# Sun-Sir/BSARec

Measured on AMD Instinct MI355X. Metric: train sequences/sec, ML-1M L=50 d=64 2-layer, higher is better.
Workload: dtype f32

## Files before the change

### bsarec_amd/csrc/fused_layer.h

```cpp
#pragma once
#include "common.h"
#include "kernels.h"
#include <type_traits>

#define FS 68
#define FU 260
#define FUSED_MAX_CB 8

struct FusedFwdP {
    const float* X; float* Xout;
    const float *sqrt_beta, *f_g, *f_b, *wq, *bq, *wk, *bk, *wv, *bv, *wo, *bo, *a_g, *a_b, *w1, *b1, *w2, *b2, *ff_g, *ff_b;
    const float* tw; const int* ids32;
    float *xhat_f, *rstd_f, *q, *k, *v, *probs, *ctx, *xhat_a, *rstd_a, *hmix, *u, *xhat_ff, *rstd_ff, *dsp;
    float* gp;
    int L, Lp, cb, heads;
    float alpha, oma, eps;
    DropP drop_f, drop_p, drop_o, drop_ff;
    float* trash;
    long long* stamps;
    const float *e_E, *e_pos, *e_g, *e_b; const int64_t* e_ids; GatherP e_gp; DropP e_drop; int e_V;
    float *e_X0, *e_xhat, *e_rstd; int* e_ids32;
    int xout_f32;
    const float* filter_cw;
};
// ... 568 lines not shown
        }
    }
    WFrag<MM, 32> wO;
    if constexpr (!FM) load_w<MM, 32>(R2_wo, wrow + 32 * grp, wO);
    lds_barrier();
    if constexpr (!FM) {
    {
        const int lr = tid >> 4, lc = (tid & 15) << 2;
#pragma unroll
        for (int r0 = 0; r0 < 64; r0 += 32) {
            const int r = r0 + lr;
            if (r < L) {
                const long e = (tok0 + r) * 64 + lc;
                ast4<BF>(R2_q, e, ld4(sQ + r * FS + lc));
                ast4<BF>(R2_k, e, ld4(sK + r * FS + lc));
                ast4<BF>(R2_v, e, f32x4{sVt[lc * FS + r], sVt[(lc + 1) * FS + r], sVt[(lc + 2) * FS + r], sVt[(lc + 3) * FS + r]});
            }
        }
    }

    STAMP(3);
    const auto R3_ctx = KARG(FusedFwdP, ctx);
    const auto R3_drop_p = KARG(FusedFwdP, drop_p);
    const auto R3_probs = KARG(FusedFwdP, probs);
    {
        const int nt = (L + 31) >> 5;
        const float sqrt_dh = sqrtf((float)DH);
        constexpr int NCT = (DH + 31) / 32;
        const int ncombo = heads * nt;
        const int pair = wave >> 1, kt = wave & 1;
        for (int c0 = 0; c0 < ncombo; c0 += 4) {
            const int combo = c0 + pair;
            const bool act = combo < ncombo && kt < nt;
            const int head = act ? combo / nt : 0, qt = act ? combo % nt : 0;
            const int query = 32 * qt + l31;
            f32x16 st;
#pragma unroll
            for (int r = 0; r < 16; ++r) st[r] = 0.f;
            float mx = -INFINITY;
            if (act) {
                mma_ll<MM, DH>(sK + (32 * kt + l31) * FS + head * DH + KH, sQ + query * FS + head * DH + KH, st);
#pragma unroll
                for (int r = 0; r < 16; ++r) {
                    const int key = 32 * kt + rho(r) + 4 * half;
                    float s = -INFINITY;
                    if (key < L) s = st[r] / sqrt_dh + ((key <= query && sIds[key] > 0) ? 0.0f : -10000.0f);
                    st[r] = s;
                    mx = fmaxf(mx, s);
                }
                mx = xor32_max(mx);
                sRed[(pair * 2 + kt) * 64 + lane] = mx;
            }
            lds_barrier();
            float sum = 0.f;
            if (act) {
                if (nt == 2) mx = fmaxf(mx, sRed[(pair * 2 + (kt ^ 1)) * 64 + lane]);
#pragma unroll
                for (int r = 0; r < 16; ++r) {
                    const int key = 32 * kt + rho(r) + 4 * half;
                    const float e = key < L ? __expf(st[r] - mx) : 0.f;
                    st[r] = e;
                    sum += e;
                }
                sum = xor32_sum(sum);
            }
            lds_barrier();
            if (act) sRed[(pair * 2 + kt) * 64 + lane] = sum;
            lds_barrier();
            if (act) {
                if (nt == 2) sum += sRed[(pair * 2 + (kt ^ 1)) * 64 + lane];
                const float inv = 1.0f / sum;
#pragma unroll
                for (int g = 0; g < 4; ++g) {
                    const int key0 = 32 * kt + 8 * g + 4 * half;
                    f32x4 p = {st[4 * g] * inv, st[4 * g + 1] * inv, st[4 * g + 2] * inv, st[4 * g + 3] * inv};
                    f32x4 m = {1.f, 1.f, 1.f, 1.f};
                    if (query < L && key0 < Lp) {
                        const long e = (((long)b * heads + head) * L + query) * Lp + key0;
                        ast4<BF>(R3_probs, e, p);
                        m = drop_mult4(R3_drop_p, dseed, (uint64_t)e >> 2);
                    }
                    p = p * m;
                    st[4 * g] = p.x; st[4 * g + 1] = p.y; st[4 * g + 2] = p.z; st[4 * g + 3] = p.w;
                }
                float* dstT = kt == 0 ? sC : sE;
#pragma unroll
                for (int ct = 0; ct < NCT; ++ct) {
                    f32x16 cacc;
#pragma unroll
                    for (int r = 0; r < 16; ++r) cacc[r] = 0.f;
                    const bool crow_ok = 32 * ct + l31 < DH;
                    const float* va = sVt + (head * DH + 32 * ct + (crow_ok ? l31 : 0)) * FS + 32 * kt + 4 * half;
                    if constexpr (MM != 0) {
#pragma unroll
                        for (int s2 = 0; s2 < 2; ++s2) {
                            f32x4 a0 = ld4(va + 16 * s2), a1 = ld4(va + 16 * s2 + 8);
                            if (!crow_ok) { a0 = f32x4{0, 0, 0, 0}; a1 = a0; }
                            if constexpr (MM == 1) {
                                const u32x4 pb = {pk_bf16(st[8 * s2], st[8 * s2 + 1]), pk_bf16(st[8 * s2 + 2], st[8 * s2 + 3]),
                                                  pk_bf16(st[8 * s2 + 4], st[8 * s2 + 5]), pk_bf16(st[8 * s2 + 6], st[8 * s2 + 7])};
                                cacc = mfma_bf16(pk8(a0, a1), pb, cacc);
                            } else {
                                cacc = mfma_x3(split3(a0, a1), split3(f32x4{st[8 * s2], st[8 * s2 + 1], st[8 * s2 + 2], st[8 * s2 + 3]},
                                                                      f32x4{st[8 * s2 + 4], st[8 * s2 + 5], st[8 * s2 + 6], st[8 * s2 + 7]}), cacc);
                            }
                        }
                    } else {
#pragma unroll
                    for (int g = 0; g < 4; ++g) {
                        f32x4 a = ld4(va + 8 * g);
                        if (!crow_ok) a = f32x4{0, 0, 0, 0};
#pragma unroll
                        for (int j = 0; j < 4; ++j)
                            cacc = __builtin_amdgcn_mfma_f32_32x32x2f32(a[j], st[4 * g + j], cacc, 0, 0, 0);
                    }
                    }
#pragma unroll
                    for (int g = 0; g < 4; ++g) {
                        const int c = 32 * ct + 8 * g + 4 * half;
                        if (c < DH)
                            st4(dstT + query * FS + head * DH + c, f32x4{cacc[4 * g], cacc[4 * g + 1], cacc[4 * g + 2], cacc[4 * g + 3]});
                    }
                }
            }
            lds_barrier();
        }
        {
            const int lr = tid >> 4, lc = (tid & 15) << 2;
#pragma unroll
            for (int r0 = 0; r0 < 64; r0 += 32) {
                const int r = r0 + lr;
                f32x4 v = {0, 0, 0, 0};
                if (r < 32 * nt) { v = ld4(sC + r * FS + lc); if (nt == 2) v += ld4(sE + r * FS + lc); }
                st4(sC + r * FS + lc, v);
                if (r < L) ast4<BF>(R3_ctx, (tok0 + r) * 64 + lc, v);
            }
        }
    }
    lds_barrier();
    }

    STAMP(4);
    const auto R4_a_b = KARG(FusedFwdP, a_b);
    const auto R4_a_g = KARG(FusedFwdP, a_g);
    const auto R4_alpha = KARG(FusedFwdP, alpha);
    const auto R4_bo = KARG(FusedFwdP, bo);
    const auto R4_drop_o = KARG(FusedFwdP, drop_o);
    const auto R4_eps = KARG(FusedFwdP, eps);
    const auto R4_hmix = KARG(FusedFwdP, hmix);
    const auto R4_oma = KARG(FusedFwdP, oma);
    const auto R4_rstd_a = KARG(FusedFwdP, rstd_a);
    const auto R4_w1 = KARG(FusedFwdP, w1);
    const auto R4_xhat_a = KARG(FusedFwdP, xhat_a);
    float ffn_bias[2];
    LnPre lnA;
    if constexpr (!FM) lnA = ln_pre(R4_bo, R4_a_g, R4_a_b, R4_drop_o, dseed, tok0);
    {
        load_w<MM, 64>(R4_w1, (long)(128 * grp + col) * 64 + KH, wA);
        ffn_bias[0] = gld(KARG(FusedFwdP, b1) + 128 * grp + col); ffn_bias[1] = gld(KARG(FusedFwdP, b1) + 128 * grp + 64 + col);
        if constexpr (!FM) {
        f32x16 acc;
#pragma unroll
        for (int r = 0; r < 16; ++r) acc[r] = 0.f;
        mma_w<MM, 32>(sC + arow + 32 * grp, wO, acc);
        float* part = grp == 0 ? sQ : sK;
#pragma unroll
        for (int r = 0; r < 16; ++r) part[(wm * 32 + rho(r) + 4 * half) * FS + col] = acc[r];
        }
    }
    if constexpr (!FM) {
    lds_barrier();
    ln_rows_64<true, BF>(lnA, sQ, sK, sX, R4_eps, sD, R4_alpha, R4_oma, tok0, L, sH, R4_hmix, R4_xhat_a, R4_rstd_a);
    lds_barrier();
    }

    STAMP(5);
    const auto R5_b1 = KARG(FusedFwdP, b1);
    const auto R5_u = KARG(FusedFwdP, u);
    const auto R5_w1 = KARG(FusedFwdP, w1);
    const auto R5_w2 = KARG(FusedFwdP, w2);
    {
        const float* sa = sH + arow;
#pragma unroll
        for (int i = 0; i < 2; ++i) {
            const int c256 = (2 * grp + i) * 64 + col;
            WFrag<MM, 64>& wcur = i ? wB : wA;
            WFrag<MM, 64>& wnxt = i ? wA : wB;
            if (i == 0) load_w<MM, 64>(R5_w1, (long)(c256 + 64) * 64 + KH, wnxt);
            else load_w<MM, 64>(R5_w2, (long)col * 256 + 128 * grp + KH, wnxt);
            f32x16 acc;
#pragma unroll
            for (int r = 0; r < 16; ++r) acc[r] = 0.f;
            mma_w<MM, 64>(sa, wcur, acc);
            const float bias = ffn_bias[i];
#pragma unroll
            for (int r = 0; r < 16; ++r) {
                const int row = wm * 32 + rho(r) + 4 * half;
                sU[row * FU + c256] = acc[r] + bias;
            }
        }
    }
    lds_barrier();

    STAMP(6);
    const auto R6_w2 = KARG(FusedFwdP, w2);
    const auto R6_u = KARG(FusedFwdP, u);
    const auto R6_gp = KARG(FusedFwdP, gp);
    const auto R7_b2 = KARG(FusedFwdP, b2);
    const auto R7_drop_ff = KARG(FusedFwdP, drop_ff);
    const auto R7_ff_b = KARG(FusedFwdP, ff_b);
    const auto R7_ff_g = KARG(FusedFwdP, ff_g);
    LnPre lnF;
    {
        for (int idx = tid; idx < 64 * 64; idx += 512) {
            const int r = idx >> 6, c4 = (idx & 63) << 2;
            const f32x4 v = ld4(sU + r * FU + c4);
            float g0, g1, g2, g3, p0, p1, p2, p3;
            gelu_both(v.x, g0, p0); gelu_both(v.y, g1, p1); gelu_both(v.z, g2, p2); gelu_both(v.w, g3, p3);
            const f32x4 g = {g0, g1, g2, g3}, gp = {p0, p1, p2, p3};
            if (r < L) { ast4<BF>(R6_u, (tok0 + r) * 256 + c4, g); ast4<BF>(R6_gp, (tok0 + r) * 256 + c4, gp); }
            st4(sU + r * FU + c4, g);
        }
        lds_barrier();
        lnF = ln_pre(R7_b2, R7_ff_g, R7_ff_b, R7_drop_ff, dseed, tok0);
        f32x16 acc;
#pragma unroll
        for (int r = 0; r < 16; ++r) acc[r] = 0.f;
        const float* sa = sU + (wm * 32 + l31) * FU + 128 * grp + KH;
        load_w<MM, 64>(R6_w2, (long)col * 256 + 128 * grp + 64 + KH, wB);
        mma_w<MM, 64>(sa, wA, acc);
        mma_w<MM, 64>(sa + 64, wB, acc);
        float* part = grp == 0 ? sX : sE;
#pragma unroll
        for (int r = 0; r < 16; ++r) part[(wm * 32 + rho(r) + 4 * half) * FS + col] = acc[r];
    }
    lds_barrier();
    STAMP(7);
    TopFwdRegs<BF> TR;
    TopFwdHelpRegs<BF> TH;
    if constexpr (TAIL) { if (wave < 4) top_fwd_prefetch<BF, KOFF, false>(TR); else top_fwd_help_prefetch<BF, KOFF>(TH); }
    const auto R7_Xout = KARG(FusedFwdP, Xout);
    const auto R7_eps = KARG(FusedFwdP, eps);
    const auto R7_rstd_ff = KARG(FusedFwdP, rstd_ff);
    const auto R7_xhat_ff = KARG(FusedFwdP, xhat_ff);
    ln_rows_64<false, BF>(lnF, sX, sE, sH, R7_eps, nullptr, 0.f, 1.f, tok0, L,
                          TAIL ? sD : nullptr, R7_Xout, R7_xhat_ff, R7_rstd_ff, KARG(FusedFwdP, xout_f32) != 0, TAIL);
    STAMP(8);
    if constexpr (TAIL) {
        lds_barrier();
        if (wave < 4) top_fwd_rest<DH, BF, KOFF, true>(TR, dseed, sD, sR, sR + TS, sR + 2 * TS, sTab, sSpec, sX, sIds);
        else top_fwd_help<DH, BF, KOFF>(TH, sD, sR, sR + TS, sX);
    }
}
#undef PTYPE

static inline size_t fused_fwd_smem_bytes() {
    return (size_t)(8 * 64 * FS + 2 * FUSED_MAX_CB * 128 + 512 + 64) * 4;
}

struct FusedBwdP {
    const float* dY; float* dX; const float* X;
    const float *sqrt_beta, *f_g, *wq, *wk, *wv, *wo, *a_g, *w1, *w2, *ff_g;
    const float* tw;
    const float *xhat_f, *rstd_f, *q, *k, *v, *probs, *xhat_a, *rstd_a, *u, *xhat_ff, *rstd_ff;
    const float* dh_slabs; int dh_nsplit; long dh_stride;
    float *dT, *dU, *dO, *dq, *dk, *dv;
    float *pg_ff, *pb_ff, *pg_a, *pb_a, *pg_f, *pb_f, *pbeta;
    int L, Lp, cb, heads;
    float alpha, oma;
    DropP drop_f, drop_p, drop_o, drop_ff;
    float* trash;
    long long* stamps;
    float* e_dz; const float *e_xhat, *e_rstd, *e_g; float *e_pg, *e_pb; DropP e_drop;
    const float* filter_cw; float* pcw;
    const float* e_dx_extra;
};


__device__ __forceinline__ void seq_partial_64(const f32x4& v, float* __restrict__ red, float* __restrict__ dst, float scale_by = 1.f,
                                               const float* __restrict__ mul = nullptr) {
    const int lr = threadIdx.x >> 4, lc = (threadIdx.x & 15) << 2;
    const int ng = blockDim.x >> 4;
    lds_barrier();
    st4(red + lr * 64 + lc, v);
    lds_barrier();
    if (threadIdx.x < 64) {
        float s = 0.f;
        for (int g = 0; g < ng; ++g) s += red[g * 64 + threadIdx.x];
        if (mul) s *= gld(mul + threadIdx.x);
        gst(dst + threadIdx.x, s * scale_by);
    }
}


template <int N>
__device__ __forceinline__ void seq_partials_64(const f32x4 (&v)[N], float* const (&red)[N], float* const (&dst)[N],
                                                float scale0 = 1.f, const float* __restrict__ mul0 = nullptr) {
    const int lr = threadIdx.x >> 4, lc = (threadIdx.x & 15) << 2;
    const int ng = blockDim.x >> 4;
    lds_barrier();
#pragma unroll
    for (int i = 0; i < N; ++i) st4(red[i] + lr * 64 + lc, v[i]);
    lds_barrier();
    const int i = threadIdx.x >> 6, c = threadIdx.x & 63;
    if (i < N) {
        const float* r = red[0];
        float* d = dst[0];
#pragma unroll
        for (int k = 1; k < N; ++k) if (i == k) { r = red[k]; d = dst[k]; }
        float s0 = 0.f, s1 = 0.f, s2 = 0.f, s3 = 0.f;
        for (int g = 0; g < ng; g += 4) {
            s0 += r[g * 64 + c]; s1 += r[(g + 1) * 64 + c]; s2 += r[(g + 2) * 64 + c]; s3 += r[(g + 3) * 64 + c];
        }
        float sum = (s0 + s1) + (s2 + s3);
        if (i == 0) { if (mul0) sum *= gld(mul0 + c); sum *= scale0; }
        gst(d + c, sum);
    }
}

template <int DH, bool BF, class HEADP, bool X3 = false, bool FM = false>
__global__ void __launch_bounds__(512) __attribute__((amdgpu_waves_per_eu(2, 2)))
fused_layer_bwd_kernel(const FusedBwdP P_unused, const HEADP H_unused) {
#define PTYPE FusedBwdP
    static_assert(!(BF && X3), "x3 products work on fp32 tensors");
    constexpr int MM = X3 ? 2 : (BF ? 1 : 0);
    static_assert(!FM || (!BF && !X3 && !IsTail<HEADP>::value), "the FMLPRec block runs in fp32, without a top-block head");
    constexpr bool HEAD = IsTail<HEADP>::value;
    constexpr unsigned KOFF = (unsigned)((sizeof(FusedBwdP) + 7) & ~(size_t)7);
    const auto R0_L = KARG(FusedBwdP, L);
    const auto R0_Lp = KARG(FusedBwdP, Lp);
    const auto R0_cb = KARG(FusedBwdP, cb);
    const auto R0_heads = KARG(FusedBwdP, heads);
    extern __shared__ __attribute__((aligned(16))) float sm[];
    constexpr int TS = 64 * FS;
    float* sAcc = sm;
    float* sT = sm + TS;
    float* sQ = sm + 2 * TS;
    float* sK = sm + 3 * TS;
    float* sV = sm + 4 * TS;
    float* sS = sm + 5 * TS;
    float* sdU = sQ;
    float* sG = sm + 6 * TS;
    float* sdF = sm + 7 * TS;
    float* sPm = sm + 8 * TS;
    float* sTab = sm + 9 * TS;
    float* sRed = sTab + FUSED_MAX_CB * 128;
    const int tid = threadIdx.x, lane = tid & 63, wave = tid >> 6;
    const int l31 = lane & 31, half = lane >> 5;
    const int grp = wave >> 2, wm = (wave >> 1) & 1, wn = wave & 1;
    const int lr = tid >> 4, lc = (tid & 15) << 2;
    const int L = R0_L, Lp = R0_Lp, heads = R0_heads, cb = R0_cb;
    const int b = blockIdx.x;
    const long tok0 = (long)b * L;
    const int col = wn * 32 + l31;
    constexpr int KHM = MM ? 8 : 4;
    const int KH = KHM * half;
    const int arow = (wm * 32 + l31) * FS + KH;
    float* const trash = KARG(FusedBwdP, trash) + 4 * lane;

    STAMP(0);
    const KernargTouch ktouch = kernarg_touch<KOFF + (unsigned)sizeof(HEADP)>();
    TopBwdRegs HR;
    TopBwdHelpRegs HH;
    if constexpr (HEAD) {
        if (wave == 0) top_bwd_prefetch<BF, KOFF>(HR);
        else if (wave < 4) {
            if (wave == 3) build_twiddle_table(KARG(FusedBwdP, tw), L, cb, sTab, 192, 64);
            top_bwd_prefetch_tile<BF, KOFF>(HR);
        } else top_bwd_help_prefetch<BF, KOFF>(HH);
    }
    const DropSeed dseed = drop_seed(KARG(FusedBwdP, drop_f));
    kernarg_touch_done(ktouch);
    const auto R1_dT = KARG(FusedBwdP, dT);
    const auto R1_dY = KARG(FusedBwdP, dY);
    const auto R1_dh_nsplit = KARG(FusedBwdP, dh_nsplit);
    const auto R1_dh_slabs = KARG(FusedBwdP, dh_slabs);
    const auto R1_dh_stride = KARG(FusedBwdP, dh_stride);
    const auto R1_drop_ff = KARG(FusedBwdP, drop_ff);
    const auto R1_ff_g = KARG(FusedBwdP, ff_g);
    const auto R1_pb_ff = KARG(FusedBwdP, pb_ff);
    const auto R1_pg_ff = KARG(FusedBwdP, pg_ff);
    const auto R1_rstd_ff = KARG(FusedBwdP, rstd_ff);
    const auto R1_tw = KARG(FusedBwdP, tw);
    const auto R1_w2 = KARG(FusedBwdP, w2);
    const auto R1_xhat_ff = KARG(FusedBwdP, xhat_ff);
    if constexpr (!FM && !HEAD) build_twiddle_table(R1_tw, L, cb, sTab);
    if constexpr (HEAD) {
        if (wave < 4) {
            top_bwd_body<DH, BF, KOFF, true>(HR, dseed, sG, sdF, sPm, sTab, sAcc, sT);
        } else {
            top_bwd_help_a<BF, KOFF>(HH, sAcc);
            f32x4 uw[16];
            top_bwd_help_b<DH, BF, KOFF>(sG, sAcc, KARG(FusedBwdP, u), uw);
#pragma unroll
            for (int i = 0; i < 16; ++i) {
                const int idx = (tid - 256) + i * 256, r = idx >> 6, c4 = (idx & 63) << 2;
                st4(sdU + r * FU + c4, r < L ? uw[i] : f32x4{0, 0, 0, 0});
            }
        }
    }
    WFrag<MM, 64> wA, wB;
    WFrag<MM, 32> wk4;
    f32x4 e_bt, e_x[2];
    load_wT<MM, 64, 256>(R1_w2, (long)KH * 256 + 128 * grp + col, wA);
    const f32x4 g = gld4(R1_ff_g + lc);
    f32x4 dy[2], xh[2];
    float rs[2];
#pragma unroll
    for (int i = 0; i < 2; ++i) {
        const int r = 32 * i + lr;
        const long e = (tok0 + r) * 64 + lc;
        dy[i] = f32x4{0, 0, 0, 0}; xh[i] = dy[i]; rs[i] = 0.f;
        if (R1_dh_slabs) {
            if (r < L) {
                if (r == L - 1)
                    for (int sp = 0; sp < R1_dh_nsplit; ++sp) dy[i] += gld4(R1_dh_slabs + sp * R1_dh_stride + (long)b * 64 + lc);
                xh[i] = ald4<BF>(R1_xhat_ff, e); rs[i] = gld(R1_rstd_ff + tok0 + r);
            }
        } else {
            const bool ok = r < L;
            const long ec = (tok0 + min(r, L - 1)) * 64 + lc;
            f32x4 d4 = {0, 0, 0, 0};
            if constexpr (!HEAD) d4 = ald4<BF>(R1_dY, ec);
            const f32x4 x4 = ald4<BF>(R1_xhat_ff, ec);
            const float r1 = gld(R1_rstd_ff + tok0 + min(r, L - 1));
            if constexpr (HEAD) d4 = ld4(sT + r * FS + lc);
            dy[i] = ok ? d4 : f32x4{0, 0, 0, 0}; xh[i] = ok ? x4 : f32x4{0, 0, 0, 0}; rs[i] = ok ? r1 : 0.f;
        }
    }
    f32x4 uv[8];
    if constexpr (!HEAD)
    {
        const float* gu = KARG(FusedBwdP, u);
#pragma unroll
        for (int i = 0; i < 8; ++i) {
            const int idx = tid + i * 512, r = idx >> 6, c4 = (idx & 63) << 2;
            uv[i] = ald4<BF>(gu, (tok0 + min(r, L - 1)) * 256 + c4);
        }
    }

    {
        f32x4 sg = {0, 0, 0, 0}, sb = sg;
#pragma unroll
        for (int i = 0; i < 2; ++i) {
            const int r = 32 * i + lr;
            const bool ok = r < L;
            const long e = (tok0 + r) * 64 + lc;
            const f32x4 gg = dy[i] * g;
            const float m1 = group_sum<16>(gg.x + gg.y + gg.z + gg.w) * (1.0f / 64.0f);
            const float m2 = group_sum<16>(gg.x * xh[i].x + gg.y * xh[i].y + gg.z * xh[i].z + gg.w * xh[i].w) * (1.0f / 64.0f);
            const f32x4 dz = rs[i] * (gg - m1 - xh[i] * m2);
            sg += dy[i] * xh[i]; sb += dy[i];
            f32x4 dt = {0, 0, 0, 0};
            if (ok) { dt = dz * drop_mult4(R1_drop_ff, dseed, (uint64_t)e >> 2); ast4<BF>(R1_dT, e, dt); }
            st4(sAcc + r * FS + lc, dz);
            st4(sT + r * FS + lc, dt);
        }
        {
            const f32x4 pv[2] = {sg, sb};
            float* const pr[2] = {sPm, sPm + 2048};
            float* const pd[2] = {R1_pg_ff + (long)b * 64, R1_pb_ff + (long)b * 64};
            seq_partials_64<2>(pv, pr, pd);
        }
    }
    if constexpr (!HEAD) {
#pragma unroll
    for (int i = 0; i < 8; ++i) {
        const int idx = tid + i * 512, r = idx >> 6, c4 = (idx & 63) << 2;
        st4(sdU + r * FU + c4, r < L ? uv[i] : f32x4{0, 0, 0, 0});
    }
    }
    lds_barrier();

    STAMP(1);
    const auto R2_dU = KARG(FusedBwdP, dU);
    const auto R2_u = KARG(FusedBwdP, u);
    const auto R2_w1 = KARG(FusedBwdP, w1);
    const auto R2_w2 = KARG(FusedBwdP, w2);
    if constexpr (MM == 0) {
        const float* sa = sT + arow;
        const int c0 = (2 * grp) * 64 + col, c1 = c0 + 64;
        load_wT<MM, 64, 256>(R2_w2, (long)KH * 256 + c1, wB);
        f32x16 acc0, acc1;
#pragma unroll
        for (int r = 0; r < 16; ++r) { acc0[r] = 0.f; acc1[r] = 0.f; }
        mma_w<MM, 64>(sa, wA, acc0);
        load_wT<MM, 64, 64>(R2_w1, (long)(128 * grp + KH) * 64 + col, wA);
#pragma unroll
        for (int r = 0; r < 16; ++r) {
            const f32x4 a = ld4(sa + 8 * (r >> 1));
            const int s0 = 2 * (r & 1);
            acc1 = __builtin_amdgcn_mfma_f32_32x32x2f32(a[s0], wB.w[r >> 1][s0], acc1, 0, 0, 0);
            acc1 = __builtin_amdgcn_mfma_f32_32x32x2f32(a[s0 + 1], wB.w[r >> 1][s0 + 1], acc1, 0, 0, 0);
            const int row = wm * 32 + rho(r) + 4 * half;
            float* pu = sdU + row * FU + c0;
            *pu = row < L ? acc0[r] * *pu : 0.f;
        }
#pragma unroll
        for (int r = 0; r < 16; ++r) {
            const int row = wm * 32 + rho(r) + 4 * half;
            float* pu = sdU + row * FU + c1;
            *pu = row < L ? acc1[r] * *pu : 0.f;
        }
    } else {
        const float* sa = sT + arow;
#pragma unroll
        for (int i = 0; i < 2; ++i) {
            const int blk = 2 * grp + i, c256 = blk * 64 + col;
            WFrag<MM, 64>& wcur = i ? wB : wA;
            WFrag<MM, 64>& wnxt = i ? wA : wB;
            if (i == 0) load_wT<MM, 64, 256>(R2_w2, (long)KH * 256 + c256 + 64, wnxt);
            else load_wT<MM, 64, 64>(R2_w1, (long)(128 * grp + KH) * 64 + col, wnxt);
            f32x16 acc;
#pragma unroll
            for (int r = 0; r < 16; ++r) acc[r] = 0.f;
            mma_w<MM, 64>(sa, wcur, acc);
#pragma unroll
            for (int r = 0; r < 16; ++r) {
                const int row = wm * 32 + rho(r) + 4 * half;
                float* pu = sdU + row * FU + c256;
                *pu = row < L ? acc[r] * *pu : 0.f;
            }
        }
    }
    lds_barrier();
    for (int idx = tid; idx < 64 * 64; idx += 512) {
        const int r = idx >> 6, c4 = (idx & 63) << 2;
        if (r < L) ast4<BF>(R2_dU, (tok0 + r) * 256 + c4, ld4(sdU + r * FU + c4));
    }

    STAMP(2);
    const auto R3_w1 = KARG(FusedBwdP, w1);
    const auto R3_wo = KARG(FusedBwdP, wo);
    WFrag<MM, 32> wO;
    f32x4 pq[2], pk[2], pv[2], xa[2], xf[2];
    float ra[2], rf[2];
    {
        f32x16 acc;
#pragma unroll
        for (int r = 0; r < 16; ++r) acc[r] = 0.f;
        const float* sa = sdU + (wm * 32 + l31) * FU + 128 * grp + KH;
        load_wT<MM, 64, 64>(R3_w1, (long)(128 * grp + 64 + KH) * 64 + col, wB);
        if constexpr (!FM) load_wT<MM, 32, 64>(R3_wo, (long)(32 * grp + KH) * 64 + col, wO);
#pragma unroll
        for (int i = 0; i < 2; ++i) {
            const int r = 32 * i + lr;
            const long ec = (tok0 + min(r, L - 1)) * 64 + lc;
            if constexpr (!FM) {
            pq[i] = ald4<BF>(KARG(FusedBwdP, q), ec); pk[i] = ald4<BF>(KARG(FusedBwdP, k), ec); pv[i] = ald4<BF>(KARG(FusedBwdP, v), ec);
            xa[i] = ald4<BF>(KARG(FusedBwdP, xhat_a), ec); ra[i] = gld(KARG(FusedBwdP, rstd_a) + tok0 + min(r, L - 1));
            }
            xf[i] = ald4<BF>(KARG(FusedBwdP, xhat_f), ec);
            rf[i] = gld(KARG(FusedBwdP, rstd_f) + tok0 + min(r, L - 1));
        }
        mma_w<MM, 64>(sa, wA, acc);
        mma_w<MM, 64>(sa + 64, wB, acc);
        float* part = grp == 0 ? sG : sdF;
#pragma unroll
        for (int r = 0; r < 16; ++r) part[(wm * 32 + rho(r) + 4 * half) * FS + col] = acc[r];
    }
    lds_barrier();

    STAMP(3);
    if constexpr (FM) {
        float* const sXin = sT;  float* const sdFm = sPm;  float* const tab = sV;  float* const spec = sG;
        const DropP drop_f = KARG(FusedBwdP, drop_f);
        const f32x4 gf = gld4(KARG(FusedBwdP, f_g) + lc);
        const float* const Xg = KARG(FusedBwdP, X);
        f32x4 sgf = {0, 0, 0, 0}, sbf = sgf;
        const f32x4 z4 = {0, 0, 0, 0};
        f32x4 dzf2[2], dF2[2], x2[2];
#pragma unroll
        for (int i = 0; i < 2; ++i) {
            const int r = 32 * i + lr;
            const bool ok = r < L;
            const long e = (tok0 + r) * 64 + lc;
            if (!ok) { xf[i] = z4; rf[i] = 0.f; }
            f32x4 dh = z4;
            if (ok) dh = ld4(sG + r * FS + lc) + ld4(sdF + r * FS + lc) + ld4(sAcc + r * FS + lc);
            const f32x4 g2 = dh * gf;
            const float n1 = group_sum<16>(g2.x + g2.y + g2.z + g2.w) * (1.0f / 64.0f);
            const float n2 = group_sum<16>(g2.x * xf[i].x + g2.y * xf[i].y + g2.z * xf[i].z + g2.w * xf[i].w) * (1.0f / 64.0f);
            dzf2[i] = rf[i] * (g2 - n1 - xf[i] * n2);
            sgf += dh * xf[i]; sbf += dh;
            dF2[i] = z4; x2[i] = z4;
            if (ok) {
                dF2[i] = dzf2[i] * drop_mult4(drop_f, dseed, (uint64_t)e >> 2);
                x2[i] = gld4(Xg + e);
                gst4(KARG(FusedBwdP, dO) + e, z4); gst4(KARG(FusedBwdP, dq) + e, z4);
                gst4(KARG(FusedBwdP, dk) + e, z4); gst4(KARG(FusedBwdP, dv) + e, z4);
            }
        }
        lds_barrier();
#pragma unroll
        for (int i = 0; i < 2; ++i) {
            const int r = 32 * i + lr;
            st4(sAcc + r * FS + lc, dzf2[i]);
            st4(sdFm + r * FS + lc, dF2[i]);
            st4(sXin + r * FS + lc, x2[i]);
        }
        build_twiddle_table(R1_tw, L, cb, tab);
        {
            const f32x4 pv[4] = {z4, z4, sgf, sbf};
            float* const pr[4] = {sQ, sQ + 2048, sK, sK + 2048};
            float* const pd[4] = {KARG(FusedBwdP, pg_a) + (long)b * 64, KARG(FusedBwdP, pb_a) + (long)b * 64,
                                  KARG(FusedBwdP, pg_f) + (long)b * 64, KARG(FusedBwdP, pb_f) + (long)b * 64};
            seq_partials_64<4>(pv, pr, pd);
        }
        lds_barrier();
        {
            const int lr16 = (tid & 255) >> 4;
            const float* srcT = grp == 0 ? sXin : sdFm;
            float* part = grp == 0 ? sQ : sK;
            float* specg = spec + grp * cb * 128;
            for (int k0 = 0; k0 < cb; k0 += 2) {
                f32x4 re[2], im[2];
#pragma unroll
                for (int j = 0; j < 2; ++j) { re[j] = z4; im[j] = z4; }
#pragma unroll
                for (int r0 = 0; r0 < 64; r0 += 16) {
                    const int t = r0 + lr16;
                    if (t < L) {
                        const f32x4 x = ld4(srcT + t * FS + lc);
#pragma unroll
                        for (int j = 0; j < 2; ++j)
                            if (k0 + j < cb) {
                                const float c = tab[2 * ((k0 + j) * 64 + t)], sn = tab[2 * ((k0 + j) * 64 + t) + 1];
                                re[j] += x * c; im[j] -= x * sn;
                            }
                    }
                }
#pragma unroll
                for (int j = 0; j < 2; ++j) {
                    st4(part + ((lr16 * 2 + j) * 2 + 0) * 64 + lc, re[j]);
                    st4(part + ((lr16 * 2 + j) * 2 + 1) * 64 + lc, im[j]);
                }
                lds_barrier();
                {
                    const int i = tid & 255;
                    const int j = i >> 7;
                    if (k0 + j < cb) {
                        float acc = 0.f;
#pragma unroll
                        for (int gq = 0; gq < 16; ++gq) acc += part[gq * 256 + i];
                        specg[(k0 + j) * 128 + (i & 127)] = acc;
                    }
                }
                lds_barrier();
            }
        }
        {
            const float* const cwp = KARG(FusedBwdP, filter_cw);
            float* const pcw = KARG(FusedBwdP, pcw) + (long)b * cb * 128;
            float* const sDs = spec + cb * 128;
            for (int i = tid; i < cb * 64; i += 512) {
                const int k = i >> 6, c = i & 63;
                const float xr = spec[k * 128 + c], xi = spec[k * 128 + 64 + c];
                const float dr = sDs[k * 128 + c], di = sDs[k * 128 + 64 + c];
                const float wr = gld(cwp + 2 * i), wi = gld(cwp + 2 * i + 1);
                const float wl = ((k == 0 || 2 * k == L) ? 1.0f : 2.0f) / (float)L;
                gst(pcw + 2 * i, wl * (dr * xr + di * xi));
                gst(pcw + 2 * i + 1, wl * (di * xr - dr * xi));
                sDs[k * 128 + c] = dr * wr + di * wi;
                sDs[k * 128 + 64 + c] = di * wr - dr * wi;
            }
        }
        lds_barrier();
        {
            float* const e_dz = KARG(FusedBwdP, e_dz);
            const float* const e_xhat = KARG(FusedBwdP, e_xhat);
            const float* const e_rstd = KARG(FusedBwdP, e_rstd);
            const DropP e_drop = KARG(FusedBwdP, e_drop);
            const float* const e_dx_extra = KARG(FusedBwdP, e_dx_extra);
            float* const dXg = KARG(FusedBwdP, dX);
            f32x4 g0 = z4, sg0 = z4, sb0 = z4;
            if (e_dz) g0 = gld4(KARG(FusedBwdP, e_g) + lc);
#pragma unroll
            for (int i = 0; i < 2; ++i) {
                const int t = 32 * i + lr;
                const bool ok = t < L;
                const long e = (tok0 + t) * 64 + lc;
                f32x4 dx = z4, xh = z4;
                float rs = 0.f;
                if (ok) {
                    dx = ld4(sAcc + t * FS + lc) + lowpass_tab(spec + cb * 128, t, lc, L, cb, tab);
                    if (e_dx_extra) dx += gld4(e_dx_extra + e);
                    if (e_dz) { xh = gld4(e_xhat + e); rs = gld(e_rstd + tok0 + t); dx = dx * drop_mult4(e_drop, dseed, (uint64_t)e >> 2); }
                    else gst4(dXg + e, dx);
                }
                if (e_dz) {
                    const f32x4 gg = dx * g0;
                    const float m1 = group_sum<16>(gg.x + gg.y + gg.z + gg.w) * (1.0f / 64.0f);
                    const float m2 = group_sum<16>(gg.x * xh.x + gg.y * xh.y + gg.z * xh.z + gg.w * xh.w) * (1.0f / 64.0f);
                    if (ok) gst4(e_dz + e, rs * (gg - m1 - xh * m2));
                    sg0 += dx * xh; sb0 += dx;
                }
            }
            float* const pbeta = KARG(FusedBwdP, pbeta) + (long)b * 64;
            if (e_dz) {
                const f32x4 pv[3] = {z4, sg0, sb0};
                float* const pr[3] = {sQ, sQ + 2048, sK};
                float* const pd[3] = {pbeta, KARG(FusedBwdP, e_pg) + (long)b * 64, KARG(FusedBwdP, e_pb) + (long)b * 64};
                seq_partials_64<3>(pv, pr, pd);
            } else if (tid < 64) gst(pbeta + tid, 0.f);
        }
        return;
    }
    const auto R4_a_g = KARG(FusedBwdP, a_g);
    const auto R4_alpha = KARG(FusedBwdP, alpha);
    const auto R4_dO = KARG(FusedBwdP, dO);
    const auto R4_drop_f = KARG(FusedBwdP, drop_f);
    const auto R4_drop_o = KARG(FusedBwdP, drop_o);
    const auto R4_f_g = KARG(FusedBwdP, f_g);
    const auto R4_k = KARG(FusedBwdP, k);
    const auto R4_oma = KARG(FusedBwdP, oma);
    const auto R4_pb_a = KARG(FusedBwdP, pb_a);
    const auto R4_pb_f = KARG(FusedBwdP, pb_f);
    const auto R4_pg_a = KARG(FusedBwdP, pg_a);
    const auto R4_pg_f = KARG(FusedBwdP, pg_f);
    const auto R4_q = KARG(FusedBwdP, q);
    const auto R4_rstd_a = KARG(FusedBwdP, rstd_a);
    const auto R4_rstd_f = KARG(FusedBwdP, rstd_f);
    const auto R4_v = KARG(FusedBwdP, v);
    const auto R4_xhat_a = KARG(FusedBwdP, xhat_a);
    const auto R4_xhat_f = KARG(FusedBwdP, xhat_f);
    {
        const f32x4 ga = gld4(R4_a_g + lc), gf = gld4(R4_f_g + lc);
        f32x4 sga = {0, 0, 0, 0}, sba = sga, sgf = sga, sbf = sga;
#pragma unroll
        for (int i = 0; i < 2; ++i) {
            const int r = 32 * i + lr;
            const f32x4 z4 = {0, 0, 0, 0};
            f32x4 q4 = pq[i], k4 = pk[i], v4 = pv[i];
            if (r >= L) { q4 = z4; k4 = z4; v4 = z4; xa[i] = z4; xf[i] = z4; ra[i] = 0.f; rf[i] = 0.f; }
            st4(sQ + r * FS + lc, q4); st4(sK + r * FS + lc, k4); st4(sV + r * FS + lc, v4);
        }
#pragma unroll
        for (int i = 0; i < 2; ++i) {
            const int r = 32 * i + lr;
            const bool ok = r < L;
            const long e = (tok0 + r) * 64 + lc;
            f32x4 dh = {0, 0, 0, 0};
            if (ok) dh = ld4(sG + r * FS + lc) + ld4(sdF + r * FS + lc) + ld4(sAcc + r * FS + lc);
            const f32x4 dya = dh * R4_oma, dyf = dh * R4_alpha;
            const f32x4 g1 = dya * ga, g2 = dyf * gf;
            const float m1 = group_sum<16>(g1.x + g1.y + g1.z + g1.w) * (1.0f / 64.0f);
            const float m2 = group_sum<16>(g1.x * xa[i].x + g1.y * xa[i].y + g1.z * xa[i].z + g1.w * xa[i].w) * (1.0f / 64.0f);
            const float n1 = group_sum<16>(g2.x + g2.y + g2.z + g2.w) * (1.0f / 64.0f);
            const float n2 = group_sum<16>(g2.x * xf[i].x + g2.y * xf[i].y + g2.z * xf[i].z + g2.w * xf[i].w) * (1.0f / 64.0f);
            const f32x4 dza = ra[i] * (g1 - m1 - xa[i] * m2), dzf = rf[i] * (g2 - n1 - xf[i] * n2);
            sga += dya * xa[i]; sba += dya; sgf += dyf * xf[i]; sbf += dyf;
            f32x4 dO = {0, 0, 0, 0}, dF = dO;
            if (ok) {
                dO = dza * drop_mult4(R4_drop_o, dseed, (uint64_t)e >> 2);
                dF = dzf * drop_mult4(R4_drop_f, dseed, (uint64_t)e >> 2);
                ast4<BF>(R4_dO, e, dO);
            }
            st4(sAcc + r * FS + lc, dza + dzf);
            st4(sT + r * FS + lc, dO);
            st4(sdF + r * FS + lc, dF);
        }
        {
            const f32x4 pv[4] = {sga, sba, sgf, sbf};
            float* const pr[4] = {sPm, sPm + 2048, sG, sG + 2048};
            float* const pd[4] = {R4_pg_a + (long)b * 64, R4_pb_a + (long)b * 64, R4_pg_f + (long)b * 64, R4_pb_f + (long)b * 64};
            seq_partials_64<4>(pv, pr, pd);
        }
    }
    lds_barrier();

    STAMP(4);
    {
        f32x16 acc;
#pragma unroll
        for (int r = 0; r < 16; ++r) acc[r] = 0.f;
        mma_w<MM, 32>(sT + arow + 32 * grp, wO, acc);
        float* part = grp == 0 ? sG : sPm;
#pragma unroll
        for (int r = 0; r < 16; ++r) part[(wm * 32 + rho(r) + 4 * half) * FS + col] = acc[r];
    }
    lds_barrier();
#pragma unroll
    for (int i = 0; i < 2; ++i) {
        const int r = 32 * i + lr;
        st4(sG + r * FS + lc, ld4(sG + r * FS + lc) + ld4(sPm + r * FS + lc));
    }
    lds_barrier();

    STAMP(5);
    const auto R6_dk = KARG(FusedBwdP, dk);
    const auto R6_dq = KARG(FusedBwdP, dq);
    const auto R6_drop_p = KARG(FusedBwdP, drop_p);
    const auto R6_dv = KARG(FusedBwdP, dv);
    const auto R6_probs = KARG(FusedBwdP, probs);
    {
        const int nt = (L + 31) >> 5;
        const float inv_sqrt_dh = 1.0f / sqrtf((float)DH);
        constexpr int NCT = (DH + 31) / 32;
        constexpr int NRES = (6 * NCT + 7) / 8;
        for (int head = 0; head < heads; ++head) {
            const int hc = head * DH;
            const int qt = (wave >> 1) & 1, kt = wave & 1;
            const int query = 32 * qt + l31;
            const bool c1 = wave < 4;
            f32x4 pp[4], mm[4];
            f32x16 da;
            float delta = 0.f;
            if (c1) {
#pragma unroll
                for (int g = 0; g < 4; ++g) {
                    const int key0 = 32 * kt + 8 * g + 4 * half;
                    pp[g] = f32x4{0, 0, 0, 0}; mm[g] = pp[g];
                    if (query < L && key0 < Lp) {
                        const long e = (((long)b * heads + head) * L + query) * Lp + key0;
                        pp[g] = ald4<BF>(R6_probs, e);
                        mm[g] = drop_mult4(R6_drop_p, dseed, (uint64_t)e >> 2);
                    }
                }
#pragma unroll
                for (int r = 0; r < 16; ++r) da[r] = 0.f;
                if (kt < nt && qt < nt)
                    mma_ll<MM, DH>(sV + (32 * kt + l31) * FS + hc + KH, sG + query * FS + hc + KH, da);
#pragma unroll
                for (int g = 0; g < 4; ++g)
#pragma unroll
                    for (int j = 0; j < 4; ++j) {
                        const float dA = da[4 * g + j] * mm[g][j];
                        delta += dA * pp[g][j];
                        da[4 * g + j] = dA;
                        sPm[(32 * kt + 8 * g + 4 * half + j) * FS + query] = pp[g][j] * mm[g][j];
                    }
                delta = xor32_sum(delta);
                sRed[(qt * 2 + kt) * 64 + lane] = delta;
            }
            lds_barrier();
            if (c1) {
                delta += sRed[(qt * 2 + (kt ^ 1)) * 64 + lane];
#pragma unroll
                for (int g = 0; g < 4; ++g)
#pragma unroll
                    for (int j = 0; j < 4; ++j)
                        sS[(32 * kt + 8 * g + 4 * half + j) * FS + query] = pp[g][j] * (da[4 * g + j] - delta) * inv_sqrt_dh;
            }
            lds_barrier();
            f32x16 res[NRES];
#pragma unroll
            for (int ti = 0; ti < NRES; ++ti) {
                const int t = wave + 8 * ti;
                f32x16 acc;
#pragma unroll
                for (int r = 0; r < 16; ++r) acc[r] = 0.f;
                if (t < 6 * NCT) {
                    const int kind = t / (2 * NCT), rt = (t / NCT) & 1, ct = t % NCT;
                    const int c = 32 * ct + l31;
                    const bool cok = c < DH;
                    const int cc = hc + (cok ? c : 0);
                    if (rt < nt) {
                        const float* bsrc = kind == 0 ? sK : kind == 1 ? sQ : sG;
                        const float* asrc = kind == 2 ? sPm : sS;
                        if constexpr (MM != 0) {
#pragma unroll 2
                            for (int s2 = 0; s2 < 2 * nt; ++s2) {
                                f32x4 a0, a1;
                                if (kind == 0) {
                                    const float* ap = asrc + (16 * s2 + KH) * FS + 32 * rt + l31;
                                    a0 = f32x4{ap[0], ap[FS], ap[2 * FS], ap[3 * FS]};
                                    a1 = f32x4{ap[4 * FS], ap[5 * FS], ap[6 * FS], ap[7 * FS]};
                                } else {
                                    const float* ap = asrc + (32 * rt + l31) * FS + 16 * s2 + KH;
                                    a0 = ld4(ap); a1 = ld4(ap + 4);
                                }
                                const float* bp = bsrc + (16 * s2 + KH) * FS + cc;
                                f32x4 b0 = {bp[0], bp[FS], bp[2 * FS], bp[3 * FS]}, b1 = {bp[4 * FS], bp[5 * FS], bp[6 * FS], bp[7 * FS]};
                                if (!cok) { b0 = f32x4{0, 0, 0, 0}; b1 = b0; }
                                if constexpr (MM == 1) acc = mfma_bf16(pk8(a0, a1), pk8(b0, b1), acc);
                                else acc = mfma_x3(split3(a0, a1), split3(b0, b1), acc);
                            }
                        } else {
#pragma unroll 4
                        for (int kb = 0; kb < 4 * nt; ++kb) {
                            f32x4 a;
                            if (kind == 0) {
                                const float* ap = asrc + (8 * kb + 4 * half) * FS + 32 * rt + l31;
                                a.x = ap[0]; a.y = ap[FS]; a.z = ap[2 * FS]; a.w = ap[3 * FS];
                            } else {
                                a = ld4(asrc + (32 * rt + l31) * FS + 8 * kb + 4 * half);
                            }
                            const float* bp = bsrc + (8 * kb + 4 * half) * FS + cc;
                            float w0 = bp[0], w1 = bp[FS], w2 = bp[2 * FS], w3 = bp[3 * FS];
                            if (!cok) { w0 = 0.f; w1 = 0.f; w2 = 0.f; w3 = 0.f; }
                            acc = __builtin_amdgcn_mfma_f32_32x32x2f32(a.x, w0, acc, 0, 0, 0);
                            acc = __builtin_amdgcn_mfma_f32_32x32x2f32(a.y, w1, acc, 0, 0, 0);
                            acc = __builtin_amdgcn_mfma_f32_32x32x2f32(a.z, w2, acc, 0, 0, 0);
                            acc = __builtin_amdgcn_mfma_f32_32x32x2f32(a.w, w3, acc, 0, 0, 0);
                        }
                        }
                    }
                }
                res[ti] = acc;
            }
            lds_barrier();
#pragma unroll
            for (int ti = 0; ti < NRES; ++ti) {
                const int t = wave + 8 * ti;
                if (t < 6 * NCT) {
                    const int kind = t / (2 * NCT), rt = (t / NCT) & 1, ct = t % NCT;
                    const int c = 32 * ct + l31;
                    if (c < DH) {
                        float* sdst = kind == 0 ? sQ : kind == 1 ? sK : sV;
#pragma unroll
                        for (int r = 0; r < 16; ++r) {
                            const int row = 32 * rt + rho(r) + 4 * half;
                            const float val = rt < nt ? res[ti][r] : 0.f;
                            sdst[row * FS + hc + c] = val;
                        }
                    }
                }
            }
            lds_barrier();
        }
        {
            const long wofs = (long)KH * 64 + col;
            if (grp == 0) { load_wT<MM, 64, 64>(KARG(FusedBwdP, wq), wofs, wA); load_wT<MM, 32, 64>(KARG(FusedBwdP, wk), wofs, wk4); }
            else { load_wT<MM, 32, 64>(KARG(FusedBwdP, wk), wofs + 32 * 64, wk4); load_wT<MM, 64, 64>(KARG(FusedBwdP, wv), wofs, wA); }
            const float* const pX = KARG(FusedBwdP, X);
            e_bt = gld4(KARG(FusedBwdP, sqrt_beta) + lc);
#pragma unroll
            for (int i = 0; i < 2; ++i) e_x[i] = ald4<BF>(pX, (tok0 + min(32 * i + lr, L - 1)) * 64 + lc);
        }
#pragma unroll
        for (int i = 0; i < 2; ++i) {
            const int r = 32 * i + lr;
            if (r < L) {
                const long e = (tok0 + r) * 64 + lc;
                ast4<BF>(R6_dq, e, ld4(sQ + r * FS + lc));
                ast4<BF>(R6_dk, e, ld4(sK + r * FS + lc));
                ast4<BF>(R6_dv, e, ld4(sV + r * FS + lc));
            }
        }
    }

    STAMP(6);
    {
        f32x16 acc;
#pragma unroll
        for (int r = 0; r < 16; ++r) acc[r] = 0.f;
        mma_w<MM, 64>((grp == 0 ? sQ : sV) + arow, wA, acc);
        mma_w<MM, 32>(sK + arow + 32 * grp, wk4, acc);
        float* part = grp == 0 ? sG : sPm;
#pragma unroll
        for (int r = 0; r < 16; ++r) part[(wm * 32 + rho(r) + 4 * half) * FS + col] = acc[r];
    }
    lds_barrier();

    STAMP(7);
    const auto R8_dX = KARG(FusedBwdP, dX);
    const auto R8_pbeta = KARG(FusedBwdP, pbeta);
    const auto R8_sqrt_beta = KARG(FusedBwdP, sqrt_beta);
    {
        float* sXin = sT;
        float* spec = sAcc;
        float* part = (grp == 0 ? sQ : sV);
        const f32x4 bt = e_bt;
        const f32x4 b2 = bt * bt, omb2 = 1.0f - b2;
        float* const e_dz = KARG(FusedBwdP, e_dz);
        const float* const e_dx_extra = KARG(FusedBwdP, e_dx_extra);
        f32x4 g0 = {0, 0, 0, 0}, e_xh[2], e_ex[2], e_dm[2];
        float e_rs[2];
#pragma unroll
        for (int i = 0; i < 2; ++i) { e_xh[i] = f32x4{0, 0, 0, 0}; e_ex[i] = e_xh[i]; e_dm[i] = e_xh[i]; e_rs[i] = 0.f; }
        if (e_dz || e_dx_extra) {
            const float* const e_xhat = KARG(FusedBwdP, e_xhat);
            const float* const e_rstd = KARG(FusedBwdP, e_rstd);
            const DropP e_drop = KARG(FusedBwdP, e_drop);
            if (e_dz) g0 = gld4(KARG(FusedBwdP, e_g) + lc);
#pragma unroll
            for (int i = 0; i < 2; ++i) {
                const int t = 32 * i + lr;
                const long e = (tok0 + min(t, L - 1)) * 64 + lc;
                if (e_dx_extra) e_ex[i] = gld4(e_dx_extra + e);
                if (e_dz) { e_xh[i] = ald4<BF>(e_xhat, e); e_rs[i] = gld(e_rstd + tok0 + min(t, L - 1)); e_dm[i] = drop_mult4(e_drop, dseed, (uint64_t)e >> 2); }
            }
        }
#pragma unroll
        for (int i = 0; i < 2; ++i) {
            const int r = 32 * i + lr;
            f32x4 x = e_x[i];
            if (r >= L) x = f32x4{0, 0, 0, 0};
            st4(sG + r * FS + lc, ld4(sG + r * FS + lc) + ld4(sPm + r * FS + lc) + ld4(sAcc + r * FS + lc));
            st4(sXin + r * FS + lc, x);
        }
        lds_barrier();
        const int lr16 = (tid & 255) >> 4;
        const float* srcT = grp == 0 ? sXin : sdF;
        float* specg = spec + grp * cb * 128;
#pragma unroll
        for (int ch = 0; ch < FUSED_MAX_CB / 4; ++ch) {
            const int k0 = 4 * ch;
            if (k0 >= cb) break;
            f32x4 re[4], im[4];
#pragma unroll
            for (int j = 0; j < 4; ++j) { re[j] = f32x4{0, 0, 0, 0}; im[j] = f32x4{0, 0, 0, 0}; }
#pragma unroll
            for (int r0 = 0; r0 < 64; r0 += 16) {
                const int t = r0 + lr16;
                if (t < L) {
                    f32x4 x = ld4(srcT + t * FS + lc);
                    if (grp == 1) x = x * omb2;
#pragma unroll
                    for (int j = 0; j < 4; ++j)
                        if (k0 + j < cb) {
                            const float c = sTab[2 * ((k0 + j) * 64 + t)], sn = sTab[2 * ((k0 + j) * 64 + t) + 1];
                            re[j] += x * c; im[j] -= x * sn;
                        }
                }
            }
#pragma unroll
            for (int j = 0; j < 4; ++j) {
                st4(part + ((lr16 * 4 + j) * 2 + 0) * 64 + lc, re[j]);
                st4(part + ((lr16 * 4 + j) * 2 + 1) * 64 + lc, im[j]);
            }
            lds_barrier();
            for (int i = tid & 255; i < 512; i += 256) {
                const int j = i >> 7, rc = i & 127;
                if (k0 + j < cb) {
                    float acc = 0.f;
#pragma unroll
                    for (int g = 0; g < 16; ++g) acc += part[g * 512 + i];
                    specg[(k0 + j) * 128 + rc] = acc;
                }
            }
            lds_barrier();
        }
        f32x4 sb = {0, 0, 0, 0}, sg0 = sb, sb0 = sb;
#pragma unroll
        for (int i = 0; i < 2; ++i) {
            const int t = 32 * i + lr;
            const bool ok = t < L;
            const long e = (tok0 + t) * 64 + lc;
            f32x4 dx = {0, 0, 0, 0}, xh = dx;
            float rs = 0.f;
            if (ok) {
                const f32x4 xv = ld4(sXin + t * FS + lc), df = ld4(sdF + t * FS + lc);
                const f32x4 lowx = lowpass_tab(spec, t, lc, L, cb, sTab);
                const f32x4 lowg = lowpass_tab(spec + cb * 128, t, lc, L, cb, sTab);
                dx = ld4(sG + t * FS + lc) + b2 * df + lowg;
                if (e_dx_extra) dx += e_ex[i];
                sb += df * (xv - lowx);
                if (e_dz) { xh = e_xh[i]; rs = e_rs[i]; dx = dx * e_dm[i]; }
                else ast4<BF>(R8_dX, e, dx);
            }
            if (e_dz) {
                const f32x4 gg = dx * g0;
                const float m1 = group_sum<16>(gg.x + gg.y + gg.z + gg.w) * (1.0f / 64.0f);
                const float m2 = group_sum<16>(gg.x * xh.x + gg.y * xh.y + gg.z * xh.z + gg.w * xh.w) * (1.0f / 64.0f);
                if (ok) gst4(e_dz + e, rs * (gg - m1 - xh * m2));
                sg0 += dx * xh; sb0 += dx;
            }
        }
        if (e_dz) {
            const f32x4 pv[3] = {sb, sg0, sb0};
            float* const pr[3] = {sQ, sQ + 2048, sQ + 4096};
            float* const pd[3] = {R8_pbeta + (long)b * 64, KARG(FusedBwdP, e_pg) + (long)b * 64, KARG(FusedBwdP, e_pb) + (long)b * 64};
            seq_partials_64<3>(pv, pr, pd, 2.0f, R8_sqrt_beta);
        } else {
            const f32x4 pv[1] = {sb};
            float* const pr[1] = {sQ};
            float* const pd[1] = {R8_pbeta + (long)b * 64};
            seq_partials_64<1>(pv, pr, pd, 2.0f, R8_sqrt_beta);
        }
    }
    STAMP(8);
}
#undef PTYPE

static inline size_t fused_bwd_smem_bytes() { return (size_t)(9 * 64 * FS + FUSED_MAX_CB * 128 + 512) * 4; }
```

Baseline: 1.648 million.

## Process two attention heads per iteration in fused backward, keep dz in registers

New measurement: 1.671 million, median of 6. 1.01x the previous value.

```diff
diff --git a/bsarec_amd/csrc/fused_layer.h b/bsarec_amd/csrc/fused_layer.h
--- a/bsarec_amd/csrc/fused_layer.h
+++ b/bsarec_amd/csrc/fused_layer.h
@@ -894,19 +894,18 @@
 #pragma unroll
     for (int i = 0; i < N; ++i) st4(red[i] + lr * 64 + lc, v[i]);
     lds_barrier();
-    const int i = threadIdx.x >> 6, c = threadIdx.x & 63;
-    if (i < N) {
-        const float* r = red[0];
-        float* d = dst[0];
-#pragma unroll
-        for (int k = 1; k < N; ++k) if (i == k) { r = red[k]; d = dst[k]; }
+    const int wv = __builtin_amdgcn_readfirstlane(threadIdx.x >> 6), c = threadIdx.x & 63;
+#pragma unroll
+    for (int i = 0; i < N; ++i) {
+        if (wv != i) continue;
+        const float* const r = red[i];
         float s0 = 0.f, s1 = 0.f, s2 = 0.f, s3 = 0.f;
         for (int g = 0; g < ng; g += 4) {
             s0 += r[g * 64 + c]; s1 += r[(g + 1) * 64 + c]; s2 += r[(g + 2) * 64 + c]; s3 += r[(g + 3) * 64 + c];
         }
         float sum = (s0 + s1) + (s2 + s3);
         if (i == 0) { if (mul0) sum *= gld(mul0 + c); sum *= scale0; }
-        gst(d + c, sum);
+        gst(dst[i] + c, sum);
     }
 }
 
@@ -1316,6 +1315,7 @@
     const auto R4_v = KARG(FusedBwdP, v);
     const auto R4_xhat_a = KARG(FusedBwdP, xhat_a);
     const auto R4_xhat_f = KARG(FusedBwdP, xhat_f);
+    f32x4 dzaf[2];
     {
         const f32x4 ga = gld4(R4_a_g + lc), gf = gld4(R4_f_g + lc);
         f32x4 sga = {0, 0, 0, 0}, sba = sga, sgf = sga, sbf = sga;
@@ -1348,7 +1348,7 @@
                 dF = dzf * drop_mult4(R4_drop_f, dseed, (uint64_t)e >> 2);
                 ast4<BF>(R4_dO, e, dO);
             }
-            st4(sAcc + r * FS + lc, dza + dzf);
+            dzaf[i] = dza + dzf;
             st4(sT + r * FS + lc, dO);
             st4(sdF + r * FS + lc, dF);
         }
@@ -1389,50 +1389,57 @@
         const int nt = (L + 31) >> 5;
         const float inv_sqrt_dh = 1.0f / sqrtf((float)DH);
         constexpr int NCT = (DH + 31) / 32;
-        constexpr int NRES = (6 * NCT + 7) / 8;
-        for (int head = 0; head < heads; ++head) {
-            const int hc = head * DH;
-            const int qt = (wave >> 1) & 1, kt = wave & 1;
-            const int query = 32 * qt + l31;
-            const bool c1 = wave < 4;
-            f32x4 pp[4], mm[4];
-            f32x16 da;
-            float delta = 0.f;
-            if (c1) {
-#pragma unroll
-                for (int g = 0; g < 4; ++g) {
-                    const int key0 = 32 * kt + 8 * g + 4 * half;
-                    pp[g] = f32x4{0, 0, 0, 0}; mm[g] = pp[g];
-                    if (query < L && key0 < Lp) {
-                        const long e = (((long)b * heads + head) * L + query) * Lp + key0;
-                        pp[g] = ald4<BF>(R6_probs, e);
-                        mm[g] = drop_mult4(R6_drop_p, dseed, (uint64_t)e >> 2);
+        constexpr int HC = DH <= 32 ? 2 : 1;
+        constexpr int NT = HC * 6 * NCT;
+        constexpr int NRES = (NT + 7) / 8;
+        for (int h0 = 0; h0 < heads; h0 += HC) {
+            {
+                const int hs = HC == 2 ? grp : 0;
+                const int head = h0 + hs;
+                const int hc = head * DH;
+                float* const tP = hs ? sT : sPm;
+                float* const tS = hs ? sAcc : sS;
+                const int qt = (wave >> 1) & 1, kt = wave & 1;
+                const int query = 32 * qt + l31;
+                f32x4 pp[4], mm[4];
+                f32x16 da;
+                float delta = 0.f;
+                if (HC == 2 || wave < 4) {
+#pragma unroll
+                    for (int g = 0; g < 4; ++g) {
+                        const int key0 = 32 * kt + 8 * g + 4 * half;
+                        pp[g] = f32x4{0, 0, 0, 0}; mm[g] = pp[g];
+                        if (query < L && key0 < Lp) {
+                            const long e = (((long)b * heads + head) * L + query) * Lp + key0;
+                            pp[g] = ald4<BF>(R6_probs, e);
+                            mm[g] = drop_mult4(R6_drop_p, dseed, (uint64_t)e >> 2);
+                        }
                     }
-                }
-#pragma unroll
-                for (int r = 0; r < 16; ++r) da[r] = 0.f;
-                if (kt < nt && qt < nt)
-                    mma_ll<MM, DH>(sV + (32 * kt + l31) * FS + hc + KH, sG + query * FS + hc + KH, da);
-#pragma unroll
-                for (int g = 0; g < 4; ++g)
-#pragma unroll
-                    for (int j = 0; j < 4; ++j) {
-                        const float dA = da[4 * g + j] * mm[g][j];
-                        delta += dA * pp[g][j];
-                        da[4 * g + j] = dA;
-                        sPm[(32 * kt + 8 * g + 4 * half + j) * FS + query] = pp[g][j] * mm[g][j];
-                    }
-                delta = xor32_sum(delta);
-                sRed[(qt * 2 + kt) * 64 + lane] = delta;
-            }
-            lds_barrier();
-            if (c1) {
-                delta += sRed[(qt * 2 + (kt ^ 1)) * 64 + lane];
-#pragma unroll
-                for (int g = 0; g < 4; ++g)
-#pragma unroll
-                    for (int j = 0; j < 4; ++j)
-                        sS[(32 * kt + 8 * g + 4 * half + j) * FS + query] = pp[g][j] * (da[4 * g + j] - delta) * inv_sqrt_dh;
+#pragma unroll
+                    for (int r = 0; r < 16; ++r) da[r] = 0.f;
+                    if (kt < nt && qt < nt)
+                        mma_ll<MM, DH>(sV + (32 * kt + l31) * FS + hc + KH, sG + query * FS + hc + KH, da);
+#pragma unroll
+                    for (int g = 0; g < 4; ++g)
+#pragma unroll
+                        for (int j = 0; j < 4; ++j) {
+                            const float dA = da[4 * g + j] * mm[g][j];
+                            delta += dA * pp[g][j];
+                            da[4 * g + j] = dA;
+                            tP[(32 * kt + 8 * g + 4 * half + j) * FS + query] = pp[g][j] * mm[g][j];
+                        }
+                    delta = xor32_sum(delta);
+                    sRed[(hs * 4 + qt * 2 + kt) * 64 + lane] = delta;
+                }
+                lds_barrier();
+                if (HC == 2 || wave < 4) {
+                    delta += sRed[(hs * 4 + qt * 2 + (kt ^ 1)) * 64 + lane];
+#pragma unroll
+                    for (int g = 0; g < 4; ++g)
+#pragma unroll
+                        for (int j = 0; j < 4; ++j)
+                            tS[(32 * kt + 8 * g + 4 * half + j) * FS + query] = pp[g][j] * (da[4 * g + j] - delta) * inv_sqrt_dh;
+                }
             }
             lds_barrier();
             f32x16 res[NRES];
@@ -1442,14 +1449,15 @@
                 f32x16 acc;
 #pragma unroll
                 for (int r = 0; r < 16; ++r) acc[r] = 0.f;
-                if (t < 6 * NCT) {
-                    const int kind = t / (2 * NCT), rt = (t / NCT) & 1, ct = t % NCT;
+                if (t < NT) {
+                    const int hs = t / (6 * NCT), u = t % (6 * NCT);
+                    const int kind = u / (2 * NCT), rt = (u / NCT) & 1, ct = u % NCT;
                     const int c = 32 * ct + l31;
                     const bool cok = c < DH;
-                    const int cc = hc + (cok ? c : 0);
+                    const int cc = (h0 + hs) * DH + (cok ? c : 0);
                     if (rt < nt) {
                         const float* bsrc = kind == 0 ? sK : kind == 1 ? sQ : sG;
-                        const float* asrc = kind == 2 ? sPm : sS;
+                        const float* asrc = kind == 2 ? (hs ? sT : sPm) : (hs ? sAcc : sS);
                         if constexpr (MM != 0) {
 #pragma unroll 2
                             for (int s2 = 0; s2 < 2 * nt; ++s2) {
@@ -1495,9 +1503,11 @@
 #pragma unroll
             for (int ti = 0; ti < NRES; ++ti) {
                 const int t = wave + 8 * ti;
-                if (t < 6 * NCT) {
-                    const int kind = t / (2 * NCT), rt = (t / NCT) & 1, ct = t % NCT;
+                if (t < NT) {
+                    const int hs = t / (6 * NCT), u = t % (6 * NCT);
+                    const int kind = u / (2 * NCT), rt = (u / NCT) & 1, ct = u % NCT;
                     const int c = 32 * ct + l31;
+                    const int hc = (h0 + hs) * DH;
                     if (c < DH) {
                         float* sdst = kind == 0 ? sQ : kind == 1 ? sK : sV;
 #pragma unroll
@@ -1579,7 +1589,7 @@
             const int r = 32 * i + lr;
             f32x4 x = e_x[i];
             if (r >= L) x = f32x4{0, 0, 0, 0};
-            st4(sG + r * FS + lc, ld4(sG + r * FS + lc) + ld4(sPm + r * FS + lc) + ld4(sAcc + r * FS + lc));
+            st4(sG + r * FS + lc, ld4(sG + r * FS + lc) + ld4(sPm + r * FS + lc) + dzaf[i]);
             st4(sXin + r * FS + lc, x);
         }
         lds_barrier();
```
